# vpc-ccg/freddie

Hardware: AMD Instinct MI355X
Metric: reads segmented/sec (whole node) (higher is better)
Workload: dtype u32

## Files before the change

freddie_amd/_lib.py:

```python
import ctypes
import os

import numpy as np

from . import build as _build

_lib = None


class SegError(RuntimeError):

    def __init__(self, msg, code=None):
        super().__init__(msg)
        self.code = code


ERR_ARG, ERR_HIP, ERR_INPUT, ERR_UNSUPPORTED = 1, 2, 3, 4


class _Params(ctypes.Structure):
    _fields_ = [
        ("sigma", ctypes.c_double), ("threshold_rate", ctypes.c_double), ("variance_factor", ctypes.c_double),
        ("max_problem_size", ctypes.c_int32), ("min_read_support_outside", ctypes.c_int32),
        ("ignore_ends", ctypes.c_int32),
# ... 8 lines not shown
        ("n_part", ctypes.c_int32),
        ("part_iv_off", ctypes.c_void_p), ("iv_start", ctypes.c_void_p), ("iv_end", ctypes.c_void_p),
        ("part_rep_off", ctypes.c_void_p), ("rep_weight", ctypes.c_void_p), ("rep_exon_off", ctypes.c_void_p),
        ("ex_ts", ctypes.c_void_p), ("ex_te", ctypes.c_void_p),
    ]


class _Sizes(ctypes.Structure):
    _fields_ = [("n_final", ctypes.c_int64), ("label_bytes", ctypes.c_int64), ("n_cand", ctypes.c_int64),
                ("n_problems", ctypes.c_int64), ("n_positions", ctypes.c_int64), ("max_problem_size", ctypes.c_int64),
                ("max_problem_reads", ctypes.c_int64)]


class _Reads(ctypes.Structure):
    _fields_ = [("n_read", ctypes.c_int64)] + [(k, ctypes.c_void_p) for k in (
        "read_part", "read_rep", "strand", "seq_len", "seq_off", "read_q_off", "qs", "qe", "cig_off", "cig_op", "cig_len", "seq_classes")]


READS_DTYPES = dict(read_part=np.int32, read_rep=np.int32, strand=np.uint8, seq_len=np.int32, seq_off=np.int64, read_q_off=np.int64,
                    qs=np.int32, qe=np.int32, cig_off=np.int64, cig_op=np.uint8, cig_len=np.int32, seq_classes=np.uint32)


class _Annot(ctypes.Structure):
    _fields_ = [("n_read", ctypes.c_int64)] + [(k, ctypes.c_void_p) for k in (
        "gap_off", "gaps", "clip_off", "clips", "poly_off", "polys", "tail", "tok_off", "tok")]


EXPORTS = ["fseg_annotate", "fseg_annotation", "fseg_abi_version", "fseg_source_hash", "fseg_results", "fseg_results_packed", "fseg_create", "fseg_destroy", "fseg_last_error", "fseg_set_params", "fseg_upload",
           "fseg_run", "fseg_sync", "fseg_get_sizes", "fseg_download", "fseg_tap", "fseg_set_profiling",
           "fseg_n_stages", "fseg_stage_name", "fseg_stage_ms", "fseg_scoring_algorithmic_bytes"]

PATHS = ("small_batch", "tiny_on", "wave_on", "fuse_on", "key32", "thr_part", "label_packed", "n_solve0", "n_solve1", "n_solve2",
         "n_wide0", "n_wide1", "n_wide2", "n_tiny", "n_work", "dpw", "wide16", "known", "solve8", "tiny_kernel", "score", "arena_dp",
         "plan", "n_arena_prob", "n_score0", "n_score1", "n_score2")

TAPS = dict(pos_off=(1, np.int64), y_raw=(2, np.int32), y=(3, np.float64), threshold=(4, np.float64),
            cand_off=(5, np.int64), cand_y=(6, np.int32), fixed=(7, np.uint8), chosen=(8, np.uint8),
            final_off=(9, np.int64), final_y=(10, np.int32), problems=(11, np.int32),
            lane_start=(12, np.int32), lane_pmax=(13, np.int32), lane_exons=(14, np.int64),
            lane_stream=(15, np.int32), exon_stream=(16, np.int32), sync=(17, np.int32), paths=(18, np.int32))


def lib_path():
    return os.environ.get("FSEG_LIB") or _build.SEG_SO


def load():
    global _lib
    if _lib is not None:
        return _lib
    path = lib_path()
    if not os.path.exists(path):
        raise SegError("%s not found: build it first (freddie_amd.build.build_seg()); there is no CPU fallback" % path)
    L = ctypes.CDLL(path)
    vp = ctypes.c_void_p
    L.fseg_abi_version.restype = ctypes.c_int
    L.fseg_create.restype = ctypes.c_int
    L.fseg_create.argtypes = [ctypes.c_int, ctypes.POINTER(vp)]
    L.fseg_destroy.restype = None
    L.fseg_destroy.argtypes = [vp]
    L.fseg_last_error.restype = ctypes.c_char_p
    L.fseg_last_error.argtypes = [vp]
    L.fseg_set_params.restype = ctypes.c_int
    L.fseg_set_params.argtypes = [vp, ctypes.POINTER(_Params)]
    L.fseg_upload.restype = ctypes.c_int
    L.fseg_upload.argtypes = [vp, ctypes.POINTER(_Batch)]
    for n in ("fseg_run", "fseg_sync"):
# ... 183 lines not shown
```

freddie_amd/csrc/freddie_seg.hip:

```cpp
#include "seg_kernels.h"

using namespace fseg;

namespace {

struct DevBuf {
    void *p = nullptr;
    size_t cap = 0;
    template <typename T> T *as() const { return reinterpret_cast<T *>(p); }
};
struct Slab {
    void *p = nullptr;
    size_t cap = 0;
};
struct HostBuf {
    void *p = nullptr;
    size_t cap = 0;
    template <typename T> T *as() const { return reinterpret_cast<T *>(p); }
};
struct Carve {
    struct Item { DevBuf *b; size_t off, bytes; };
    std::vector<Item> items;
    size_t total = 0;
    size_t add(DevBuf &b, size_t bytes) {
// ... 10 lines not shown
enum Stage { ST_HIST, ST_SMOOTH, ST_THRESHOLD, ST_CANDIDATES, ST_FIX, ST_SCORE_PREP, ST_SCORE, ST_DP, ST_REFINE, ST_FINAL, ST_LABEL, ST_COUNT,
             ST_GRAPH_PRE = ST_COUNT, ST_GRAPH_POST, ST_REPORTED };
const char *kStageNames[ST_REPORTED] = {"histogram", "smooth", "threshold", "candidates", "fix_split", "scoring_prep",
                                        "interval_scoring", "dp", "refine", "final_positions", "labels", "graph_pre",
                                        "graph_post"};

enum : unsigned {
    SEG_PRE1 = 1u,
    SEG_PRE2 = 2u,
    SEG_SCORE = 4u,
    SEG_POST1 = 8u,
    SEG_POST2 = 16u,
    SEG_STATUS = 32u,
    SEG_ALL = 63u,
};

}

hipError_t fseg_sort_pairs(void *tmp, size_t *tmp_bytes, const unsigned long long *keys_in, unsigned long long *keys_out,
                           const int *vals_in, int *vals_out, size_t n, unsigned end_bit, hipStream_t stream);

struct fseg_ctx {
    int device = 0;
    hipStream_t stream = nullptr;
    std::string err;
    bool have_params = false, have_batch = false, ran = false, pending = false;
    bool fetched = false;
    fseg_params P{};
    std::vector<double> w_main, w_refine, h_table;
    int n_part = 0;
    i64 K = 0, R = 0, I = 0, NPOS = 0, LANES = 0;
    i64 max_part_pos = 0;
    int thr_part = -1;
    i64 max_part_lanes = 0;
    int n_tiles = 0;
    bool expanded = false;
    std::vector<i64> part_iv_off, part_rep_off;
    Slab slab_in, slab_pos, slab_arena;
    HostBuf h_stage;
    HostBuf h_res;
    size_t res_off[4] = {0, 0, 0, 0};
    std::vector<i64> res_pfo;
    DevBuf d_labels;
    DevBuf d_packed;
    int fetched_packed = -1;
    bool label_packed_ok = true;
    bool label_has2 = false;
    bool run_label_packed = false;
    bool labels_unpacked = false;
    DevBuf d_sort_tmp;
    DevBuf d_part_iv_off, d_part_rep_off, d_part_lane_off, d_iv_start, d_iv_end, d_pos_off, d_iv_part,
        d_rep_exon_off, d_rep_weight, d_ex_ts, d_ex_te, d_tile_desc, d_iv_tile0, d_blk_iv0, d_rb_part, d_rb_r0, d_rb_sum, d_rb_base, d_rb_max, d_rb_cmax,
        d_hc_part, d_hc_p0, d_hc_n, d_hc_glo, d_hc_ghi;
    DevBuf d_lane_ex, d_lane_start, d_lane_pmax, d_hc_llo, d_hc_lhi, d_key_a, d_key_b, d_val_a, d_val_b, d_rep_last;
    DevBuf d_lane_lx, d_lex, d_rb_esum, d_rb_ebase;
    i64 max_rep_exons = 0;
    DevBuf d_w_main, d_w_refine, d_h_table, d_thr_tab;
    DevBuf d_bits;
    DevBuf d_y_raw, d_y, d_v, d_scan_state, d_bsum, d_bsum_side, d_g, d_pk, d_pf, d_kp;
    int n_hist_chunks = 0;
    DevBuf d_voff, d_chunk_off, d_csum, d_mean, d_thr, d_label_off, d_part_has2;
    int n_rep_blocks = 0;
    DevBuf d_cand_off, d_cand_y, d_fixed0, d_added, d_fixed, d_chosen, d_final_off, d_final_y, d_final_pos, d_final_iv, d_col_thr,
        d_col_zero;
    DevBuf d_tile_defer;
    DevBuf d_blk_pre, d_tile_tot, d_seg_iv, d_seg_prev, d_rseg_c, d_cand_pn, d_cand_ll, d_cand_ln, d_cand_wide, d_prob_bs;
// ... 44 lines not shown
    static constexpr i64 kProbSelfMax = 4 * kProbBlock;
    bool prob_self_scan = false;
    i64 scan_single_max = 512;
    bool force_scan_stall = false;
    hipGraph_t graph[2] = {nullptr, nullptr};
    hipGraphExec_t graph_exec[2] = {nullptr, nullptr};
    bool profile_plain = false;
    int n_graphs = 0;
    bool last_sized = false;
    hipEvent_t ev_b[ST_COUNT] = {}, ev_e[ST_COUNT] = {};
    hipEvent_t ev_g[4] = {};
    float stage_ms[ST_REPORTED] = {};
    static constexpr int kSide = 3, kForkEvents = 32;
    hipStream_t side[kSide] = {};
    hipEvent_t fj[kForkEvents] = {};
    bool use_fork = true;
    bool force_key64 = false;
    bool wide_by_seen = false;
    char score_plan[32] = "gM|W|hB|gST";
    bool use_wave = true;
    bool use_fuse = true;
    int fuse_lanes = kFuseLanesDefault;
    bool wide_solve = true;
    bool fuse_on = true;
    bool counts_known = false;
    i64 n_solve[3] = {0, 0, 0}, n_cls_work[4] = {0, 0, 0, 0}, n_dp_cls[3] = {0, 0, 0}, n_arena_prob = 0, n_tiny = 0;
    i64 n_wide[3] = {0, 0, 0};
    i64 max_ln = 0;
    i64 tiny_from = 256;
    bool trace = false;
    bool force_global_sort = false;
    enum { PATH_SMALL_BATCH, PATH_TINY_ON, PATH_WAVE_ON, PATH_FUSE_ON, PATH_KEY32, PATH_THR_PART, PATH_LABEL_PACKED, PATH_N_SOLVE,
           PATH_N_WIDE = PATH_N_SOLVE + 3, PATH_N_TINY = PATH_N_WIDE + 3, PATH_N_WORK, PATH_DPW, PATH_WIDE16, PATH_KNOWN, PATH_SOLVE8,
           PATH_TINY_KERNEL, PATH_SCORE, PATH_ARENA_DP, PATH_PLAN, PATH_N_ARENA_PROB, PATH_N_SCORE, PATH_WORDS = PATH_N_SCORE + 3 };
    int paths[PATH_WORDS] = {};
    DevBuf d_an_in, d_an_work, d_an_out;
    HostBuf h_an_in, h_an;
    bool have_annot = false;
    fseg_annot annot{};
};

namespace {

int fail(fseg_ctx *c, int code, const char *fmt, ...) {
    char buf[512];
    va_list ap;
    va_start(ap, fmt);
    vsnprintf(buf, sizeof buf, fmt, ap);
    va_end(ap);
    if (c) c->err = buf;
    if (code == FSEG_ERR_HIP) (void)hipGetLastError();
    return code;
}
thread_local std::string g_create_error;

#define HIP_TRY(c, expr)                                                                         \
    do {                                                                                         \
        hipError_t e__ = (expr);                                                                 \
        if (e__ != hipSuccess) return fail((c), FSEG_ERR_HIP, "%s: %s", #expr, hipGetErrorString(e__)); \
    } while (0)
#define TRY(expr) do { int rc__ = (expr); if (rc__) return rc__; } while (0)

static bool g_ablate_dp = false;
static std::atomic<int> g_in_flight[64];
static std::atomic<int> g_live[64];
static std::atomic<const fseg_ctx *> g_owner[64];
static void set_in_flight(fseg_ctx *c, bool on);
// ... 196 lines not shown
    };
    auto launch_fork_waiters = [&]() {
        if (!dev_sync) return;
        for (int k = 1; k < ps.n_seg; ++k) if (dev_side(k))
            hipLaunchKernelGGL(k_wait_word, dim3(1), dim3(64), 0, c->side[ps.side_of[k]], st, &sw->emit_gen, 1u, sync_gen, kSyncTicks);
    };
    const i64 avg_len = NPOS / (K > 0 ? K : 1);
    const int iv_threads = avg_len > 65536 ? 1024 : (avg_len > 16384 ? 256 : 64);
    int tile_grid = grid_for(c->n_tiles, 1, 16384);
    const i64 scan_nb = scan_blocks(NPOS);
    const int scan_grid = scan_nb > 0 ? (int)scan_nb : 1;
    u64 *scan_state = c->d_scan_state.as<u64>();
    const bool scan_single = scan_nb <= c->scan_single_max;
    int *bsum = scan_single ? nullptr : c->d_bsum.as<int>();
    int *bsum_side = scan_single ? nullptr : c->d_bsum_side.as<int>();
    auto scan_counts = [&](hipStream_t q, int *bs, const unsigned *flags, u64 *total_dev, i64 *off_last) {
        if (scan_single) return;
        hipLaunchKernelGGL(k_scan1, dim3(grid_for(scan_nb, 1, 4096)), dim3(256), 0, q, flags, NPOS, bs);
        hipLaunchKernelGGL(k_scan2, dim3(1), dim3(kScan2Threads), 0, q, bs, scan_nb, total_dev, off_last);
    };
    int work_grid = grid_for(c->work_cap, 1, 4096);
    ProblemArrays pr{c->d_prob_iv.as<int>(), c->d_prob_start.as<int>(), c->d_prob_n.as<int>(),
                     c->d_prob_pair_off.as<i64>(), c->d_prob_tri_off.as<i64>(), c->d_prob_flags.as<int>(),
                     c->d_prob_chain.as<int>(), c->d_prob_cov_off.as<i64>(), c->d_prob_lane_lo.as<int>(),
                     c->d_prob_lane_n.as<int>()};
    const int pg = grid_for(NPOS / 8 / kProbBlock + 1, 1, 1024);
    i64 *prob_bs = (c->prob_self_scan && !sized) ? nullptr : c->d_prob_bs.as<i64>();
    if (do_pre1) {
    {
        const i64 nw = 3 * (i64)flag_words(NPOS);
        hipLaunchKernelGGL(k_clear, dim3(grid_for(nw / 4 + 1, 256, 2048)), dim3(256), 0, s, st, c->d_bits.as<unsigned>(), nw);
    }
    begin(ST_HIST);
    hipLaunchKernelGGL(k_hist, dim3(grid_for(c->n_hist_chunks, 1, 16384)), dim3(512), 0, s, c->n_hist_chunks,
                       c->d_hc_part.as<int>(), c->d_hc_p0.as<i64>(), c->d_hc_n.as<int>(), c->d_hc_glo.as<int>(),
                       c->d_hc_ghi.as<int>(), c->d_hc_llo.as<i64>(), c->d_hc_lhi.as<i64>(), c->d_part_iv_off.as<i64>(), c->d_iv_start.as<int>(), c->d_iv_end.as<int>(),
                       c->d_pos_off.as<i64>(), c->d_part_lane_off.as<i64>(), c->d_lane_lx.as<int2>(),
                       c->d_lane_start.as<int>(), c->d_lane_pmax.as<int>(),
                       c->d_lex.as<int2>(), c->P.ignore_ends, c->d_y_raw.as<int>(), st,
                       scan_state, scan_single ? scan_nb * 3 : 0);
    end(ST_HIST); begin(ST_SMOOTH);
#define FSEG_LAUNCH_SMOOTH(RV)                                                                                         \
    hipLaunchKernelGGL(k_smooth<RV>, dim3(tile_grid), dim3(kSmoothThreads), 0, s, c->n_tiles, c->d_tile_desc.as<TileDesc>(),      \
                       c->d_y_raw.as<int>(), c->d_w_main.as<double>(),                                                 \
                       c->P.radius_main, c->d_y.as<double>(), flag_pos_bits,                           \
                       flag_cand_bits, c->d_blk_pre.as<int>(), c->d_tile_tot.as<int>(), c->d_tile_defer.as<int>())
    if (c->P.radius_main == 20) { FSEG_LAUNCH_SMOOTH(20); }
    else if (c->P.radius_main == 12) { FSEG_LAUNCH_SMOOTH(12); }
    else { FSEG_LAUNCH_SMOOTH(0); }
#undef FSEG_LAUNCH_SMOOTH
    end(ST_SMOOTH);
    {
    hipStream_t q = fork(0);
    if (stage_events && c->profile_all) (void)hipEventRecord(c->ev_b[ST_THRESHOLD], q);
    const bool thr_part_fits = c->max_part_pos <= (i64)kThrPartMaxChunks * 8192;
    const bool thr_part = thr_part_fits && (c->thr_part == 1 || (c->thr_part < 0 && n_part >= 64));
    if (thr_part) {
        c->paths[fseg_ctx::PATH_THR_PART] = 1;
        hipLaunchKernelGGL(k_thr_part, dim3(grid_for(n_part, 1, 4096)), dim3(512), 0, q, n_part, c->d_part_iv_off.as<i64>(), c->d_pos_off.as<i64>(), NPOS,
                           flag_pos_bits, c->d_y.as<double>(), c->d_v.as<double>(), c->P.variance_factor, c->d_mean.as<double>(), c->d_thr.as<double>());
    } else {
    c->paths[fseg_ctx::PATH_THR_PART] = 0;
    scan_counts(q, bsum_side, flag_pos_bits, &st->n_vals, nullptr);
    hipLaunchKernelGGL(k_scan_emit<kEmitValues>, dim3(scan_grid), dim3(256), 0, q, flag_pos_bits, NPOS,
                       bsum_side, scan_state, &st->n_vals, (i64 *)nullptr, &st->err, c->d_y.as<double>(), c->d_v.as<double>(), K, c->d_pos_off.as<i64>(),
                       c->d_iv_start.as<int>(), c->d_blk_iv0.as<int>(), (int *)nullptr, (int *)nullptr, (i64 *)nullptr,
                       c->force_scan_stall ? 1 : 0, (int *)nullptr);
    hipLaunchKernelGGL(k_voff, dim3(grid_for(n_part + 1, 1, 2048)), dim3(64), 0, q, n_part, c->d_part_iv_off.as<i64>(),
                       c->d_pos_off.as<i64>(), NPOS, flag_pos_bits, bsum_side, scan_state, &st->n_vals,
                       c->d_voff.as<i64>());
    hipLaunchKernelGGL(k_vplan, dim3(1), dim3(256), 0, q, n_part, c->d_part_iv_off.as<i64>(), c->d_pos_off.as<i64>(), NPOS,
                       c->d_voff.as<i64>(), c->d_chunk_off.as<i64>(), st, c->chunk_cap);
    int chunk_grid = grid_for(c->chunk_cap, 1, 4096);
// ... 43 lines not shown
    begin(ST_SCORE_PREP);
    hipLaunchKernelGGL(k_prob_emit, dim3(pg), dim3(256), 0, s, st, c->d_cand_pn.as<int>(), c->d_cand_ll.as<int>(),
                       c->d_cand_ln.as<int>(), c->d_seg_iv.as<int>(), c->d_cand_off.as<i64>(), prob_bs,
                       pr, c->prob_cap, c->d_work_pc.as<int2>(), c->d_cls_items.as<int4>(),
                       c->work_cap, c->d_dp_items.as<int>(), c->d_prob_desc.as<ProbDesc>(), c->d_iv_start.as<int>(),
                       c->d_iv_part.as<int>(), c->d_part_lane_off.as<i64>(), split, c->d_solve_items.as<int>(), c->d_solve_desc.as<ProbDesc>(),
                       c->d_wide_items.as<int>(), c->d_wide_all.as<int>(), c->d_cand_wide.as<unsigned char>(),
                       dev_sync ? sw : (SyncWords *)nullptr, sync_gen);
    launch_fork_waiters();
    if (c->prob_cap > 0 && any_arena) {
        if (stage_events && do_score) { end(ST_SCORE_PREP); begin(ST_SCORE); score_begun = true; }
        const int cov_blocks = work_grid < 2048 ? work_grid : 2048;
        const int pt_blocks = c->small_batch ? grid_for(c->prob_cap, 1, 512) : 0;
        if (!pt_blocks)
            hipLaunchKernelGGL(k_pair_thresholds, dim3(grid_for(c->prob_cap, 1, 2048)), dim3(256), 0, s, st, pr,
                               c->d_prob_desc.as<ProbDesc>(), c->prob_cap, c->d_cand_off.as<i64>(), c->d_cand_y.as<int>(),
                               c->d_h_table.as<double>(), c->P.h_len,
                               c->P.threshold_rate, c->d_pair_thr.as<int2>(), c->pair_cap, c->d_amb.as<unsigned>(),
                               c->d_out.as<unsigned>(), c->tri_cap);
        hipLaunchKernelGGL(k_cov, dim3(cov_blocks + pt_blocks), dim3(kLaneChunk), 0, s, st,
                           c->d_prob_desc.as<ProbDesc>(), c->prob_cap, c->d_work_pc.as<int2>(), c->work_cap, c->d_cand_off.as<i64>(),
                           c->d_cand_y.as<int>(), c->d_iv_start.as<int>(), c->d_lane_lx.as<int2>(),
                           c->d_lex.as<int2>(),
                           c->d_cov.as<unsigned>(), c->cov_cap, c->d_work_active.as<unsigned char>(),
                           cov_blocks, pr, c->d_h_table.as<double>(), c->P.h_len, c->P.threshold_rate, c->d_pair_thr.as<int2>(),
                           c->pair_cap, c->d_amb.as<unsigned>(), c->d_out.as<unsigned>(), c->tri_cap);
    }
    if (!score_begun) end(ST_SCORE_PREP);
    }
    if (do_score && !score_begun) begin(ST_SCORE);
    int *const census = c->paths;
    if (do_score) {
        for (int w = 0; w < fseg_ctx::PATH_WORDS; ++w)
            if (w != fseg_ctx::PATH_THR_PART && w != fseg_ctx::PATH_LABEL_PACKED && w != fseg_ctx::PATH_ARENA_DP) census[w] = 0;
        census[fseg_ctx::PATH_SMALL_BATCH] = c->small_batch; census[fseg_ctx::PATH_TINY_ON] = c->tiny_on; census[fseg_ctx::PATH_WAVE_ON] = wave;
        census[fseg_ctx::PATH_FUSE_ON] = c->use_fuse && c->fuse_on; census[fseg_ctx::PATH_KNOWN] = known; census[fseg_ctx::PATH_PLAN] = plan != nullptr;
    }
    if (do_score && c->prob_cap > 0) {
        const bool sfork = any_arena;
        hipStream_t qt = (tiny_max > 0 && sfork) ? fork(2) : s;
#ifdef FSEG_SCORE_TIMING
#define FSEG_TARG , c->d_tacc.as<unsigned long long>()
#else
#define FSEG_TARG
#endif
#ifndef FSEG_WG_SMALL
#define FSEG_WG_SMALL 4096
#endif
#ifndef FSEG_WG_MID
#define FSEG_WG_MID 2048
#endif
#ifndef FSEG_WG_TINY
#define FSEG_WG_TINY 4096
#endif
#define FSEG_LAUNCH_SCORE(Q, NMV, CLS, MAXWG)                                                                           \
        do { note_score(CLS);                                                                                                  \
        hipLaunchKernelGGL(k_score<NMV>, dim3(work_grid < (MAXWG) ? work_grid : (MAXWG)), dim3(ScoreCfg<NMV>::kThreads),  \
                           score_lds_for((NMV) == kNMax ? c->nm_big : (NMV), (NMV) + 1), Q, st, CLS,                                 \
                           ((NMV) == kNMax ? c->nm_big : (NMV)), pr, c->prob_cap, c->d_cls_items.as<int4>(),              \
                           c->d_prob_desc.as<ProbDesc>(), c->work_cap, c->d_cand_off.as<i64>(),                         \
                           c->d_cand_y.as<int>(), c->d_work_active.as<unsigned char>(), c->d_cov.as<unsigned>(),        \
                           c->cov_cap, c->d_pair_thr.as<int2>(), c->pair_cap, c->d_out.as<unsigned>(), c->tri_cap,      \
                           c->d_amb.as<unsigned>() FSEG_TARG); } while (0)
        auto wide_n = [&](int cls, size_t cnt_bytes) -> i64 { return (known && cls >= 0 && cls < 3 && cnt_bytes == 2) ? c->n_wide[cls] : -1; };
#define FSEG_SOLVE_N(CNT, CLS, N_ITEMS) (wide_n(CLS, sizeof(CNT)) >= 0 ? wide_n(CLS, sizeof(CNT)) : (i64)(N_ITEMS))
#define FSEG_SOLVE_WIDE(CNT, CLS) (wide_n(CLS, sizeof(CNT)) >= 0 ? c->d_wide_items.as<int>() : (const int *)nullptr)
#define FSEG_SOLVE_ARGS(NMV, CNT, CLS)                                                                                      \
// ... 645 lines not shown
        e = hipFuncSetAttribute(reinterpret_cast<const void *>(k_score_huge), hipFuncAttributeMaxDynamicSharedMemorySize,
                                (int)kHugeScoreLds);
    {
        auto lds_attr = [&](const void *f, size_t bytes) { if (e == hipSuccess) e = hipFuncSetAttribute(f, hipFuncAttributeMaxDynamicSharedMemorySize, (int)bytes); };
        lds_attr(reinterpret_cast<const void *>(k_solve<kNMax, unsigned char, int, false>), solve_lds_for(kNMax, kNMax + 1, 1));
        lds_attr(reinterpret_cast<const void *>(k_solve<kNMax, unsigned char, i64, false>), solve_lds_for(kNMax, kNMax + 1, 1));
        lds_attr(reinterpret_cast<const void *>(k_solve<kNMax, unsigned short, int, false>), solve_lds_for(kNMax, kNMax + 1, 2));
        lds_attr(reinterpret_cast<const void *>(k_solve<kNMax, unsigned short, i64, false>), solve_lds_for(kNMax, kNMax + 1, 2));
        lds_attr(reinterpret_cast<const void *>(k_solve<kNMax, unsigned char, int, true>), solve_lds_for(kNMax, kNMax + 1, 1));
        lds_attr(reinterpret_cast<const void *>(k_solve<kNMax, unsigned short, int, true>), solve_lds_for(kNMax, kNMax + 1, 2));
        lds_attr(reinterpret_cast<const void *>(k_dpw<kNMax, unsigned char, int, 64>), dpw_lds_for(kNMax, 4, 1));
        lds_attr(reinterpret_cast<const void *>(k_dpw<kNMax, unsigned short, int, 64>), dpw_lds_for(kNMax, 4, 2));
        lds_attr(reinterpret_cast<const void *>(k_dpw<kNMax, unsigned char, i64, 64>), dpw_lds_for(kNMax, 8, 1));
        lds_attr(reinterpret_cast<const void *>(k_dpw<kNMax, unsigned short, i64, 64>), dpw_lds_for(kNMax, 8, 2));
        lds_attr(reinterpret_cast<const void *>(k_dpw<kNMax, unsigned char, int, 512>), dpw_lds_for(kNMax, 4, 1));
        lds_attr(reinterpret_cast<const void *>(k_dpw<kNMax, unsigned short, int, 512>), dpw_lds_for(kNMax, 4, 2));
        lds_attr(reinterpret_cast<const void *>(k_dpw<kNMax, unsigned char, i64, 512>), dpw_lds_for(kNMax, 8, 1));
        lds_attr(reinterpret_cast<const void *>(k_dpw<kNMax, unsigned short, i64, 512>), dpw_lds_for(kNMax, 8, 2));
    }
    if (e == hipSuccess)
        e = hipFuncSetAttribute(reinterpret_cast<const void *>(k_dp_huge), hipFuncAttributeMaxDynamicSharedMemorySize,
                                (int)kHugeDpLds);
    if (e != hipSuccess) {
        g_create_error = std::string("context creation failed: ") + hipGetErrorString(e);
        if (c->counted_live) g_live[device].fetch_sub(1);
        delete c;
        return FSEG_ERR_HIP;
    }
    c->d_status.cap = sizeof(Status); c->d_prep.cap = sizeof(PrepStatus); c->d_tacc.cap = kTaccBytes; c->d_sync.cap = sizeof(SyncWords);
    auto flag = [](const char *name) { const char *v = getenv(name); return v && v[0] == '1'; };
    { const char *v = getenv("FSEG_DEV_SYNC"); if (v && v[0] == '0') c->dev_sync = false; }
    if (flag("FSEG_LABEL_BYTES")) c->label_packed_ok = false;
    { const char *v = getenv("FSEG_THR_PART"); if (v && (v[0] == '0' || v[0] == '1')) c->thr_part = v[0] - '0'; }
    { const char *v = getenv("FSEG_SYNC_TICKS"); if (v && v[0] && atoll(v) > 0) c->sync_ticks = (unsigned)atoll(v); }
    if (flag("FSEG_NO_GRAPH")) c->use_graph = false;
    if (flag("FSEG_NO_FORK")) c->use_fork = false;
    if (flag("FSEG_NO_FUSE")) c->use_fuse = false;
    if (flag("FSEG_NO_WAVE")) c->use_wave = false;
    if (flag("FSEG_FORCE_KEY64")) c->force_key64 = true;
    if (flag("FSEG_WIDE_BY_SEEN")) c->wide_by_seen = true;
    if (const char *e = getenv("FSEG_SPLIT_DP")) c->split_dp = atoi(e) & 15;
    if (const char *e = getenv("FSEG_SCORE_PLAN")) snprintf(c->score_plan, sizeof c->score_plan, "%s", e);
    {
        int seen[4] = {0, 0, 0, 0};
        static const char kinds[] = "BMST";
        for (const char *q = c->score_plan; *q; ++q) { const char *at = strchr(kinds, *q); if (at) ++seen[at - kinds]; }
        int bars = 0;
        for (const char *q = c->score_plan; *q; ++q) bars += *q == '|';
        if (seen[0] != 1 || seen[1] != 1 || seen[2] != 1 || seen[3] != 1 || bars > fseg_ctx::kSide) c->score_plan[0] = 0;
    }
    { const char *v = getenv("FSEG_FUSE_LANES"); if (v && v[0] && atoi(v) > 0 && atoi(v) <= kFuseLanesWide) c->fuse_lanes = atoi(v); }
    if (flag("FSEG_NO_SIZED")) c->use_sized = false;
    if (flag("FSEG_TRACE")) c->trace = true;
    if (flag("FSEG_GLOBAL_SORT")) c->force_global_sort = true;
    if (flag("FSEG_FORCE_SCAN_STALL")) c->force_scan_stall = true;
    { const char *tf = getenv("FSEG_TINY_FROM"); if (tf && tf[0]) c->tiny_from = atoll(tf); }
    { const char *sm = getenv("FSEG_SCAN_SINGLE_MAX"); if (sm && sm[0]) c->scan_single_max = atoll(sm); }
    *out = c;
    return FSEG_OK;
}

void fseg_destroy(fseg_ctx *c) {
    if (!c) return;
    set_in_flight(c, false);
    release_device(c);
    if (c->counted_live) { g_live[c->device].fetch_sub(1); c->counted_live = false; }
// ... 72 lines not shown
    const i64 K = b->part_iv_off[np], R = b->part_rep_off[np];
    if (b->part_iv_off[0] != 0 || b->part_rep_off[0] != 0 || b->rep_exon_off[0] != 0)
        return fail(c, FSEG_ERR_ARG, "fseg_upload: offsets must start at 0");
    if (K <= 0 || R < 0) return fail(c, FSEG_ERR_ARG, "fseg_upload: bad offsets");
    const i64 I = b->rep_exon_off[R];
    if (I < 0) return fail(c, FSEG_ERR_ARG, "rep_exon_off not monotone");
    if (I >= 0x7fffffffLL) return fail(c, FSEG_ERR_UNSUPPORTED, "batch has %lld exons; split it (limit 2^31-1 per upload)", (long long)I);
    i64 NPOS = 0, n_tiles = 0, lanes = 0, n_rep_blocks = 0, max_part_reps = 0, max_rep_exons = 0;
    bool expanded = false;
    for (int p = 0; p < np; ++p) {
        const i64 k0 = b->part_iv_off[p], k1 = b->part_iv_off[p + 1];
        if (k1 <= k0) return fail(c, FSEG_ERR_INPUT, "partition %d has no intervals", p);
        if (b->part_rep_off[p + 1] < b->part_rep_off[p]) return fail(c, FSEG_ERR_ARG, "part_rep_off not monotone");
        for (i64 k = k0; k < k1; ++k) {
            if (!(b->iv_start[k] < b->iv_end[k])) return fail(c, FSEG_ERR_INPUT, "partition %d: interval with start >= end (py/freddie_segment.py:140)", p);
            if (k > k0 && !(b->iv_end[k - 1] < b->iv_start[k])) return fail(c, FSEG_ERR_INPUT, "partition %d: intervals overlap or are unordered (py/freddie_segment.py:138)", p);
            const i64 len = (i64)b->iv_end[k] - b->iv_start[k] + 1;
            NPOS += len;
            n_tiles += (len + kSmoothTile - 1) / kSmoothTile;
        }
        n_rep_blocks += (b->part_rep_off[p + 1] - b->part_rep_off[p] + 255) / 256;
        if (b->part_rep_off[p + 1] - b->part_rep_off[p] > max_part_reps) max_part_reps = b->part_rep_off[p + 1] - b->part_rep_off[p];
    }
    if (NPOS >= 0x7fffffffLL) return fail(c, FSEG_ERR_UNSUPPORTED, "batch has %lld positions; split it (limit 2^31-1 per upload)", (long long)NPOS);
    for (i64 r = 0; r < R; ++r) {
        const int w = b->rep_weight[r];
        if (w < 1) return fail(c, FSEG_ERR_INPUT, "rep %lld has weight %d (< 1)", (long long)r, w);
        if (w != 1) expanded = true;
        lanes += w;
        if (b->rep_exon_off[r + 1] < b->rep_exon_off[r]) return fail(c, FSEG_ERR_ARG, "rep_exon_off not monotone");
        if (b->rep_exon_off[r + 1] - b->rep_exon_off[r] > max_rep_exons) max_rep_exons = b->rep_exon_off[r + 1] - b->rep_exon_off[r];
    }
    if (lanes >= 0x7fffffffLL) return fail(c, FSEG_ERR_UNSUPPORTED, "batch has %lld reads; split it (limit 2^31-1 per upload)", (long long)lanes);
    int hist_chunk = kHistChunk;
    while (hist_chunk > 1024 && NPOS / hist_chunk < 512) hist_chunk >>= 1;
    i64 n_chunks = 0;
    {
        i64 k = 0, pos = 0;
        for (int p = 0; p < np; ++p) {
            i64 Pp = 0;
            for (k = b->part_iv_off[p]; k < b->part_iv_off[p + 1]; ++k) Pp += (i64)b->iv_end[k] - b->iv_start[k] + 1;
            n_chunks += (Pp + hist_chunk - 1) / hist_chunk;
            pos += Pp;
        }
        (void)pos;
    }
    const i64 nb = scan_blocks(NPOS);
    if (n_tiles >= 0x7fffffffLL || n_chunks >= 0x7fffffffLL) return fail(c, FSEG_ERR_UNSUPPORTED, "batch too large");
    Carve in;
    in.add(c->d_part_iv_off, ((size_t)np + 1) * 8);
    in.add(c->d_part_rep_off, ((size_t)np + 1) * 8);
    in.add(c->d_part_lane_off, ((size_t)np + 1) * 8);
    in.add(c->d_iv_start, (size_t)K * 4);
    in.add(c->d_iv_end, (size_t)K * 4);
    in.add(c->d_pos_off, ((size_t)K + 1) * 8);
    in.add(c->d_iv_part, (size_t)K * 4);
    in.add(c->d_iv_tile0, (size_t)K * 4);
    in.add(c->d_tile_desc, (size_t)n_tiles * sizeof(TileDesc));
    in.add(c->d_blk_iv0, ((size_t)nb + 1) * 4);
    in.add(c->d_rb_part, (size_t)n_rep_blocks * 4);
    in.add(c->d_rb_r0, (size_t)n_rep_blocks * 4);
    in.add(c->d_hc_part, (size_t)n_chunks * 4);
    in.add(c->d_hc_p0, (size_t)n_chunks * 8);
    in.add(c->d_hc_n, (size_t)n_chunks * 4);
    in.add(c->d_hc_glo, (size_t)n_chunks * 4);
    in.add(c->d_hc_ghi, (size_t)n_chunks * 4);
    in.add(c->d_rep_exon_off, ((size_t)R + 1) * 8);
// ... 48 lines not shown
            }
            for (i64 r = b->part_rep_off[p]; r < b->part_rep_off[p + 1]; r += 256) { h_rb_part[rb] = p; h_rb_r0[rb] = (int)r; ++rb; }
            for (i64 r = b->part_rep_off[p]; r < b->part_rep_off[p + 1]; ++r) l += b->rep_weight[r];
            h_lane_off[p + 1] = l;
            if (l - h_lane_off[p] > c->max_part_lanes) c->max_part_lanes = l - h_lane_off[p];
            const i64 P0 = h_pos_off[k0], P1 = h_pos_off[k1];
            if (P1 - P0 > c->max_part_pos) c->max_part_pos = P1 - P0;
            i64 k = k0;
            for (i64 q0 = P0; q0 < P1; q0 += hist_chunk) {
                const i64 q1 = std::min<i64>(q0 + hist_chunk, P1) - 1;
                while (h_pos_off[k + 1] <= q0) ++k;
                i64 kk = k;
                while (h_pos_off[kk + 1] <= q1) ++kk;
                h_hc_part[ch] = p; h_hc_p0[ch] = q0; h_hc_n[ch] = (int)(q1 - q0 + 1);
                h_hc_glo[ch] = b->iv_start[k] + (int)(q0 - h_pos_off[k]);
                h_hc_ghi[ch] = b->iv_start[kk] + (int)(q1 - h_pos_off[kk]);
                ++ch;
            }
        }
        h_blk[nb] = (int)(K - 1);
    }
    const double t_tables = tk.ms();
    memcpy(host_of(c->d_part_iv_off), b->part_iv_off, ((size_t)np + 1) * 8);
    memcpy(host_of(c->d_part_rep_off), b->part_rep_off, ((size_t)np + 1) * 8);
    memcpy(host_of(c->d_iv_start), b->iv_start, (size_t)K * 4);
    memcpy(host_of(c->d_iv_end), b->iv_end, (size_t)K * 4);
    memcpy(host_of(c->d_rep_exon_off), b->rep_exon_off, ((size_t)R + 1) * 8);
    memcpy(host_of(c->d_rep_weight), b->rep_weight, (size_t)R * 4);
    memcpy(host_of(c->d_ex_ts), b->ex_ts, (size_t)I * 4);
    memcpy(host_of(c->d_ex_te), b->ex_te, (size_t)I * 4);
    const double t_copy = tk.ms();
    c->n_part = np; c->K = K; c->R = R; c->I = I; c->NPOS = NPOS; c->LANES = lanes; c->expanded = expanded;
    if (c->max_part_lanes > lanes) c->max_part_lanes = lanes;
    c->n_tiles = (int)n_tiles; c->n_hist_chunks = (int)n_chunks; c->n_rep_blocks = (int)n_rep_blocks; c->max_rep_exons = max_rep_exons;
    c->part_iv_off.assign(b->part_iv_off, b->part_iv_off + np + 1);
    c->part_rep_off.assign(b->part_rep_off, b->part_rep_off + np + 1);
    hipStream_t s = c->stream;
    HIP_TRY(c, hipMemcpyAsync(c->slab_in.p, stage, up_bytes, hipMemcpyHostToDevice, s));
    {
        PrepStatus init;
        init.err = 0; init.pad = 0;
        for (int q = 0; q < 4; ++q) init.bad_rep[q] = 0x7fffffffffffffffLL;
        *c->h_prep = init;
        HIP_TRY(c, hipMemcpyAsync(c->d_prep.p, c->h_prep, sizeof(PrepStatus), hipMemcpyHostToDevice, s));
        c->prep_checked = false;
    }
    if (R > 0) {
        hipLaunchKernelGGL(k_prep_reps, dim3(grid_for(n_rep_blocks, 1, 65536)), dim3(256), 0, s, (int)n_rep_blocks, c->d_rb_part.as<int>(),
                           c->d_rb_r0.as<int>(), c->d_part_rep_off.as<i64>(), c->d_part_iv_off.as<i64>(), c->d_iv_start.as<int>(),
                           c->d_iv_end.as<int>(), c->d_rep_exon_off.as<i64>(), c->d_ex_ts.as<int>(), c->d_ex_te.as<int>(),
                           c->d_key_a.as<u64>(), c->d_val_a.as<int>(), c->d_rep_last.as<int>(), c->d_prep.as<PrepStatus>());
        const bool sort_here = max_part_reps <= kLaneSortMax && !c->force_global_sort;
        if (!sort_here) {
            unsigned end_bit = 33;
            while (end_bit < 64 && ((u64)np >> (end_bit - 32)) != 0) ++end_bit;
            size_t tmp_bytes = 0;
            HIP_TRY(c, fseg_sort_pairs(nullptr, &tmp_bytes, c->d_key_a.as<u64>(), c->d_key_b.as<u64>(), c->d_val_a.as<int>(), c->d_val_b.as<int>(),
                                       (size_t)R, end_bit, s));
            TRY(ensure(c, c->d_sort_tmp, tmp_bytes));
            HIP_TRY(c, fseg_sort_pairs(c->d_sort_tmp.p, &tmp_bytes, c->d_key_a.as<u64>(), c->d_key_b.as<u64>(), c->d_val_a.as<int>(),
                                       c->d_val_b.as<int>(), (size_t)R, end_bit, s));
        }
        if (sort_here) {
            hipLaunchKernelGGL(k_lanes, dim3(grid_for(np, 1, 65536)), dim3(256), 0, s, np, c->d_part_rep_off.as<i64>(), c->d_part_lane_off.as<i64>(),
                               c->d_key_b.as<u64>(), c->d_val_b.as<int>(), c->d_rep_weight.as<int>(), c->d_rep_last.as<int>(),
                               c->d_rep_exon_off.as<i64>(), c->d_lane_ex.as<longlong2>(), c->d_lane_start.as<int>(), c->d_lane_pmax.as<int>(),
                               1, c->d_key_a.as<u64>(), c->d_ex_ts.as<int>(), c->d_ex_te.as<int>(), c->d_lane_lx.as<int2>(), c->d_lex.as<int2>());
// ... 624 lines not shown
```

freddie_amd/csrc/seg_common.h:

```cpp
#pragma once
#include <hip/hip_runtime.h>
#include <type_traits>
#include <hsa/hsa.h>
#include <hsa/hsa_ext_amd.h>
#include <chrono>
#include <algorithm>
#include <atomic>
#include <mutex>
#include <cmath>
#include <cstdarg>
#include <cstdio>
#include <cstdlib>
#include <cstring>
#include <string>
#include <vector>

#include "freddie_seg.h"

namespace fseg {


typedef long long i64;

typedef unsigned long long u64;
// ... 141 lines not shown
    if (i < 0) i += p;
    return i < n ? i : p - 1 - i;
}


__device__ __forceinline__ void label_thresholds(i64 L, const double *h_table, int h_len, double tau, int *hi_out,
                                                 int *lo_out) {
    double h = L < (i64)h_len ? h_table[L] : tau;
    double l = 1.0 - h;
    double dL = (double)L;
    i64 v = (i64)floor(h * dL);
    if (v < 0) v = 0;
    while (v > 0 && (double)(v - 1) / dL > h) --v;
    while (!((double)v / dL > h) && v <= L + 1) ++v;
    *hi_out = (int)v;
    i64 u = (i64)ceil(l * dL);
    if (u > L) u = L;
    while (u >= 0 && !((double)u / dL < l)) --u;
    while ((double)(u + 1) / dL < l && u < L) ++u;
    *lo_out = (int)u;
}


constexpr int kThrTab = 8192;

__device__ __forceinline__ void label_thresholds_tab(i64 L, const int2 *tab, const double *h_table, int h_len, double tau,
                                                     int *hi_out, int *lo_out) {
    if (L < (i64)kThrTab) { const int2 t = tab[L]; *hi_out = t.x; *lo_out = t.y; }
    else label_thresholds(L, h_table, h_len, tau, hi_out, lo_out);
}


constexpr int kHistChunk = 8192;

constexpr int kHistIv = 1024;


template <int NW = 0> __device__ __forceinline__ int wg_exclusive_scan(int v, int *lds, int *total);


__device__ __forceinline__ void lds_barrier() {
    __builtin_amdgcn_fence(__ATOMIC_RELEASE, "workgroup", "local");
    __builtin_amdgcn_s_barrier();
    __builtin_amdgcn_fence(__ATOMIC_ACQUIRE, "workgroup", "local");
}

template <int NW = 0>
__device__ __forceinline__ int wg_exclusive_scan_lds(int v, int *lds , int *total) {
    int lane = threadIdx.x & 63, wave = threadIdx.x >> 6;
    const int nw = NW > 0 ? NW : (int)((blockDim.x + 63) >> 6);
    int x = v;
    for (int d = 1; d < 64; d <<= 1) {
        int y = __shfl_up(x, d);
        if (lane >= d) x += y;
    }
    lds_barrier();
    if (lane == 63) lds[wave] = x;
    lds_barrier();
    int off = 0, tot = 0;
    for (int w = 0; w < nw; ++w) {
        int sv = lds[w];
        if (w < wave) off += sv;
        tot += sv;
    }
    *total = tot;
    return off + x - v;
// ... 1031 lines not shown
```

freddie_amd/csrc/seg_front.hip:

```cpp
#include "seg_kernels.h"

#include <type_traits>

namespace fseg {

__global__ void __launch_bounds__(256) k_thr_table(const double *h_table, int h_len, double tau, int2 *tab) {
    for (int L = blockIdx.x * blockDim.x + threadIdx.x; L < kThrTab; L += gridDim.x * blockDim.x) {
        int hi = 0x7fffffff, lo = -1;
        if (L >= 1) label_thresholds((i64)L, h_table, h_len, tau, &hi, &lo);
        tab[L] = make_int2(hi, lo);
    }
}

__global__ void __launch_bounds__(512) k_hist(int n_chunks, const int *chunk_part, const i64 *chunk_p0, const int *chunk_n,
                                              const int *chunk_glo, const int *chunk_ghi, const i64 *chunk_lane_lo,
                                              const i64 *chunk_lane_hi, const i64 *part_iv_off,
                                              const int *iv_start, const int *iv_end, const i64 *pos_off,
                                              const i64 *part_lane_off, const int2 *__restrict__ lane_lx, const int *lane_start,
                                              const int *lane_pmax, const int2 *__restrict__ lex,
                                              int ignore_ends, int *y_raw, Status *st, u64 *zero_ptr, i64 zero_n) {
    __shared__ int hist[kHistChunk];
    __shared__ int ivs_s[kHistIv], ive_s[kHistIv], base_s[kHistIv];
    for (i64 i = (i64)blockIdx.x * blockDim.x + threadIdx.x; i < zero_n; i += (i64)gridDim.x * blockDim.x) zero_ptr[i] = 0;
    for (int ch = blockIdx.x; ch < n_chunks; ch += gridDim.x) {
        const int part = chunk_part[ch];
        const i64 p0 = chunk_p0[ch];
        const int np = chunk_n[ch];
        const int g_lo = chunk_glo[ch], g_hi = chunk_ghi[ch];
        const i64 k0 = part_iv_off[part], k1 = part_iv_off[part + 1];
        __syncthreads();
        for (int i = threadIdx.x; i < np; i += blockDim.x) hist[i] = 0;
        const i64 lo = chunk_lane_lo[ch], hi = chunk_lane_hi[ch];
        const int nk = (int)(k1 - k0);
        const bool cached = nk <= kHistIv;
        if (cached)
            for (int i = threadIdx.x; i < nk; i += blockDim.x) {
                ivs_s[i] = iv_start[k0 + i]; ive_s[i] = iv_end[k0 + i];
                base_s[i] = (int)(pos_off[k0 + i] - p0) - iv_start[k0 + i];
            }
        __syncthreads();
        const int sub = threadIdx.x & 7;
        const int G8 = blockDim.x >> 3;
        auto count_exon = [&](i64 e, i64 e0, i64 e1, int ts, int te) {
            if (te < g_lo || ts > g_hi) return;
            int kl = 0;
            bool ok;
            int base;
            if (cached) {
                int a2 = 0, b2 = nk;
                while (b2 - a2 > 1) { int m = (a2 + b2) >> 1; if (ivs_s[m] <= ts) a2 = m; else b2 = m; }
                kl = a2;
                ok = ts >= ivs_s[kl] && ts <= ive_s[kl] && te <= ive_s[kl];
                base = base_s[kl];
            } else {
                ok = ts >= iv_start[k0];
                i64 k = k0;
                if (ok) { k = k0 + last_le(iv_start + k0, k1 - k0, ts); ok = ts <= iv_end[k] && te <= iv_end[k]; }
                base = (int)(pos_off[k] - p0) - iv_start[k];
            }
            if (!ok) { atomicOr(&st->err, kErrExonInterval); return; }
            if (!(ignore_ends && e == e0) && ts >= g_lo && ts <= g_hi) atomicAdd(&hist[base + ts], 1);
            if (!(ignore_ends && e == e1 - 1) && te >= g_lo && te <= g_hi) atomicAdd(&hist[base + te], 1);
        };
        for (i64 l0 = lo + (threadIdx.x >> 3); l0 < hi; l0 += 4 * (i64)G8) {
            int2 ex[4], x0[4];
#pragma unroll
            for (int u = 0; u < 4; ++u) { const i64 l = l0 + (i64)u * G8; ex[u] = lane_lx[l < hi ? l : l0]; }
#pragma unroll
            for (int u = 0; u < 4; ++u) {
                const int e = ex[u].x + sub < ex[u].y ? ex[u].x + sub : ex[u].x;
                x0[u] = lex[e];
            }
#pragma unroll
            for (int u = 0; u < 4; ++u) {
                if (l0 + (i64)u * G8 >= hi) break;
                const i64 e0 = ex[u].x, e1 = ex[u].y;
                if (e0 + sub < e1) count_exon(e0 + sub, e0, e1, x0[u].x, x0[u].y);
                for (i64 e = e0 + sub + 8; e < e1; e += 8) { const int2 x = lex[e]; count_exon(e, e0, e1, x.x, x.y); }
            }
        }
        __syncthreads();
        for (int i = threadIdx.x; i < np; i += blockDim.x) y_raw[p0 + i] = hist[i];
    }
}

template <int R>
#ifndef FSEG_SMOOTH_OCC
#define FSEG_SMOOTH_OCC 6
#endif
__global__ void __launch_bounds__(kSmoothThreads, FSEG_SMOOTH_OCC) k_smooth(int n_tiles, const TileDesc *__restrict__ tiles,
                                                const int *__restrict__ y_raw, const double *__restrict__ w_g, int radius_rt,
                                                double *y_out, unsigned *flag_pos, unsigned *flag_cand, int *blk_pre, int *tile_tot,
                                                int *tile_defer) {
    __shared__ int xs[kSmoothTile + 2 * kMaxRadius];
    __shared__ unsigned tw_c[kSmoothTile / 32 + 1], tw_p[kSmoothTile / 32 + 1];
    __shared__ int defer_s;
    __shared__ int blk_s[kSmoothTile / kSumBlock];
    __shared__ double ws[kMaxRadius + 1];
    __shared__ double ys[kSmoothTile];
    const int radius = R > 0 ? R : radius_rt;
    const int span = kSmoothTile + 2 * radius;
    constexpr int kStage = R > 0 ? (kSmoothTile + 2 * R + kSmoothThreads - 1) / kSmoothThreads : kSmoothStage;
    for (int j = threadIdx.x; j <= radius; j += blockDim.x) ws[j] = w_g[j];
    const int G = gridDim.x;
    auto load_counts = [&](const TileDesc &d, int *v) {
        const int len_d = __builtin_amdgcn_readfirstlane(d.len), y0_d = __builtin_amdgcn_readfirstlane(d.y0);
        const int yb = y0_d - radius + (int)threadIdx.x;
        const int *src = y_raw + (((i64)__builtin_amdgcn_readfirstlane((int)(d.base >> 32)) << 32) | (unsigned)__builtin_amdgcn_readfirstlane((int)d.base));
        if (R > 0 && y0_d + kSmoothTile + radius <= len_d) {
            static_assert(R <= kSmoothThreads, "a tile's left halo lies in the first staged element of each thread");
#pragma unroll
            for (int e = 0; e < kStage; ++e) {
                const int idx = e * kSmoothThreads + threadIdx.x;
                const int y = yb + e * kSmoothThreads;
                const int r = e == 0 && y < 0 ? -1 - y : y;
// ... 488 lines not shown
__global__ void k_vsum_part(int n_part, const i64 *voff, const i64 *chunk_off, const double *csum0, const double *csum1,
                            double vf, double *mean, double *thr, i64 chunk_cap) {
    for (int p = blockIdx.x * blockDim.x + threadIdx.x; p < n_part; p += gridDim.x * blockDim.x) {
        i64 c0 = chunk_off[p], c1 = chunk_off[p + 1];
        if (c1 > chunk_cap) c1 = chunk_cap;
        double n = (double)(voff[p + 1] - voff[p]);
        double s0 = 0.0, s1 = 0.0;
        for (i64 c = c0; c < c1; ++c) {
            s0 = (c == c0) ? csum0[c] : __dadd_rn(s0, csum0[c]);
            s1 = (c == c0) ? csum1[c] : __dadd_rn(s1, csum1[c]);
        }
        const double mu = s0 / n;
        mean[p] = mu;
        thr[p] = __dadd_rn(mu, __dmul_rn(vf, __dsqrt_rn(s1 / n)));
    }
}

__global__ void __launch_bounds__(256) k_peaks_edges(int n_tiles, const TileDesc *tiles, const int *tile_defer, const double *x,
                                                     unsigned *flag, int *part_has2, int n_part) {
    if (blockIdx.x == 0) for (int p = threadIdx.x; p < n_part; p += blockDim.x) part_has2[p] = 0;
    for (int t = blockIdx.x * blockDim.x + threadIdx.x; t < n_tiles; t += gridDim.x * blockDim.x) {
        const TileDesc d = tiles[t];
        const i64 first = d.base + d.y0, last = d.base + d.len - 1;
        const i64 tile_last = first + kSmoothTile - 1;
        if (d.y0 > 0 && first < last) peak_from(first, last, x, flag);
        if (tile_last < last && kSmoothTile > 1) peak_from(tile_last, last, x, flag);
        const int df = tile_defer[t];
        if (df >= 0) peak_from(first + df, last, x, flag);
    }
}


__attribute__((used)) static const void *const kInstances[] = {
    reinterpret_cast<const void *>(&k_smooth<20>),
    reinterpret_cast<const void *>(&k_smooth<12>),
    reinterpret_cast<const void *>(&k_smooth<0>),
    reinterpret_cast<const void *>(&k_scan_emit<kEmitValues>),
    reinterpret_cast<const void *>(&k_scan_emit<kEmitPositions>),
};

}
```

freddie_amd/csrc/seg_kernels.h:

```cpp
#pragma once
#include "seg_common.h"

namespace fseg {

__global__ void __launch_bounds__(256) k_thr_table(const double *h_table, int h_len, double tau, int2 *tab);

__global__ void __launch_bounds__(512) k_hist(int n_chunks, const int *chunk_part, const i64 *chunk_p0, const int *chunk_n,
                                              const int *chunk_glo, const int *chunk_ghi, const i64 *chunk_lane_lo,
                                              const i64 *chunk_lane_hi, const i64 *part_iv_off,
                                              const int *iv_start, const int *iv_end, const i64 *pos_off,
                                              const i64 *part_lane_off, const int2 *__restrict__ lane_lx, const int *lane_start,
                                              const int *lane_pmax, const int2 *__restrict__ lex,
                                              int ignore_ends, int *y_raw, Status *st, u64 *zero_ptr, i64 zero_n);

template <int R>
#ifndef FSEG_SMOOTH_OCC
#define FSEG_SMOOTH_OCC 6
#endif
__global__ void __launch_bounds__(kSmoothThreads, FSEG_SMOOTH_OCC) k_smooth(int n_tiles, const TileDesc *__restrict__ tiles,
                                                const int *__restrict__ y_raw, const double *__restrict__ w_g, int radius_rt,
                                                double *y_out, unsigned *flag_pos, unsigned *flag_cand, int *blk_pre, int *tile_tot,
                                                int *tile_defer);

__global__ void __launch_bounds__(256) k_clear(Status *st, unsigned *bits, i64 n_words);

__global__ void __launch_bounds__(256) k_scan1(const unsigned *flags, i64 n, int *bsum);

__global__ void __launch_bounds__(kScan2Threads) k_scan2(int *bsum, i64 nb, u64 *total_out, i64 *off_last );

template <int MODE>
__global__ void __launch_bounds__(256) k_scan_emit(const unsigned *flags, i64 n, const int *bsum ,
                                                   u64 *state, u64 *total_out, i64 *off_last ,
                                                   unsigned *err, const double *y,
                                                   double *v, i64 K, const i64 *pos_off, const int *iv_start,
                                                   const int *blk_iv0, int *out_y, int *out_pos, i64 *out_off,
                                                   int force_stall , int *out_iv );

__global__ void __launch_bounds__(64) k_voff(int n_part, const i64 *part_iv_off, const i64 *pos_off, i64 n_pos,
                                             const unsigned *flags, const int *bsum , const u64 *state, const u64 *total, i64 *voff);
// ... 229 lines not shown
```

Baseline: 577.6 million.

## Pack histogram counters into 16-bit halves to double shared-memory chunk size

Adds a templated k_hist variant that stores two 16-bit position counters per shared-memory word, which allows a 16384-position chunk in the same LDS footprint. The host checks at upload whether any partition could exceed 65535 overlapping exon ends (via a sort of weighted endpoints) and falls back to 32-bit counters if so. Larger chunks mean fewer chunks and less per-chunk overhead (interval caching, zeroing), and zeroing uses 16-byte stores. The cost is a host-side sort per large partition during upload, plus extra unpacking on write-out.

```diff
diff --git a/freddie_amd/_lib.py b/freddie_amd/_lib.py
--- a/freddie_amd/_lib.py
+++ b/freddie_amd/_lib.py
@@ -64,7 +64,7 @@
 
 PATHS = ("small_batch", "tiny_on", "wave_on", "fuse_on", "key32", "thr_part", "label_packed", "n_solve0", "n_solve1", "n_solve2",
          "n_wide0", "n_wide1", "n_wide2", "n_tiny", "n_work", "dpw", "wide16", "known", "solve8", "tiny_kernel", "score", "arena_dp",
-         "plan", "n_arena_prob", "n_score0", "n_score1", "n_score2")
+         "plan", "n_arena_prob", "n_score0", "n_score1", "n_score2", "hist16")
 
 TAPS = dict(pos_off=(1, np.int64), y_raw=(2, np.int32), y=(3, np.float64), threshold=(4, np.float64),
             cand_off=(5, np.int64), cand_y=(6, np.int32), fixed=(7, np.uint8), chosen=(8, np.uint8),
diff --git a/freddie_amd/csrc/freddie_seg.hip b/freddie_amd/csrc/freddie_seg.hip
--- a/freddie_amd/csrc/freddie_seg.hip
+++ b/freddie_amd/csrc/freddie_seg.hip
@@ -66,6 +66,8 @@
     i64 K = 0, R = 0, I = 0, NPOS = 0, LANES = 0;
     i64 max_part_pos = 0;
     int thr_part = -1;
+    int hist16 = -1;
+    bool hist_packed = false;
     i64 max_part_lanes = 0;
     int n_tiles = 0;
     bool expanded = false;
@@ -176,7 +178,7 @@
     bool force_global_sort = false;
     enum { PATH_SMALL_BATCH, PATH_TINY_ON, PATH_WAVE_ON, PATH_FUSE_ON, PATH_KEY32, PATH_THR_PART, PATH_LABEL_PACKED, PATH_N_SOLVE,
            PATH_N_WIDE = PATH_N_SOLVE + 3, PATH_N_TINY = PATH_N_WIDE + 3, PATH_N_WORK, PATH_DPW, PATH_WIDE16, PATH_KNOWN, PATH_SOLVE8,
-           PATH_TINY_KERNEL, PATH_SCORE, PATH_ARENA_DP, PATH_PLAN, PATH_N_ARENA_PROB, PATH_N_SCORE, PATH_WORDS = PATH_N_SCORE + 3 };
+           PATH_TINY_KERNEL, PATH_SCORE, PATH_ARENA_DP, PATH_PLAN, PATH_N_ARENA_PROB, PATH_N_SCORE, PATH_HIST16 = PATH_N_SCORE + 3, PATH_WORDS };
     int paths[PATH_WORDS] = {};
     DevBuf d_an_in, d_an_work, d_an_out;
     HostBuf h_an_in, h_an;
@@ -439,13 +441,18 @@
         hipLaunchKernelGGL(k_clear, dim3(grid_for(nw / 4 + 1, 256, 2048)), dim3(256), 0, s, st, c->d_bits.as<unsigned>(), nw);
     }
     begin(ST_HIST);
-    hipLaunchKernelGGL(k_hist, dim3(grid_for(c->n_hist_chunks, 1, 16384)), dim3(512), 0, s, c->n_hist_chunks,
-                       c->d_hc_part.as<int>(), c->d_hc_p0.as<i64>(), c->d_hc_n.as<int>(), c->d_hc_glo.as<int>(),
-                       c->d_hc_ghi.as<int>(), c->d_hc_llo.as<i64>(), c->d_hc_lhi.as<i64>(), c->d_part_iv_off.as<i64>(), c->d_iv_start.as<int>(), c->d_iv_end.as<int>(),
-                       c->d_pos_off.as<i64>(), c->d_part_lane_off.as<i64>(), c->d_lane_lx.as<int2>(),
-                       c->d_lane_start.as<int>(), c->d_lane_pmax.as<int>(),
-                       c->d_lex.as<int2>(), c->P.ignore_ends, c->d_y_raw.as<int>(), st,
-                       scan_state, scan_single ? scan_nb * 3 : 0);
+#define FSEG_LAUNCH_HIST(BITS)                                                                                         \
+    hipLaunchKernelGGL(k_hist<BITS>, dim3(grid_for(c->n_hist_chunks, 1, 16384)), dim3(512), 0, s, c->n_hist_chunks,   \
+                       c->d_hc_part.as<int>(), c->d_hc_p0.as<i64>(), c->d_hc_n.as<int>(), c->d_hc_glo.as<int>(),       \
+                       c->d_hc_ghi.as<int>(), c->d_hc_llo.as<i64>(), c->d_hc_lhi.as<i64>(), c->d_part_iv_off.as<i64>(), c->d_iv_start.as<int>(), c->d_iv_end.as<int>(), \
+                       c->d_pos_off.as<i64>(), c->d_part_lane_off.as<i64>(), c->d_lane_lx.as<int2>(),                  \
+                       c->d_lane_start.as<int>(), c->d_lane_pmax.as<int>(),                                            \
+                       c->d_lex.as<int2>(), c->P.ignore_ends, c->d_y_raw.as<int>(), st,                                \
+                       scan_state, scan_single ? scan_nb * 3 : 0)
+    c->paths[fseg_ctx::PATH_HIST16] = c->hist_packed;
+    if (c->hist_packed) { FSEG_LAUNCH_HIST(16); }
+    else { FSEG_LAUNCH_HIST(32); }
+#undef FSEG_LAUNCH_HIST
     end(ST_HIST); begin(ST_SMOOTH);
 #define FSEG_LAUNCH_SMOOTH(RV)                                                                                         \
     hipLaunchKernelGGL(k_smooth<RV>, dim3(tile_grid), dim3(kSmoothThreads), 0, s, c->n_tiles, c->d_tile_desc.as<TileDesc>(),      \
@@ -555,7 +562,7 @@
     int *const census = c->paths;
     if (do_score) {
         for (int w = 0; w < fseg_ctx::PATH_WORDS; ++w)
-            if (w != fseg_ctx::PATH_THR_PART && w != fseg_ctx::PATH_LABEL_PACKED && w != fseg_ctx::PATH_ARENA_DP) census[w] = 0;
+            if (w != fseg_ctx::PATH_THR_PART && w != fseg_ctx::PATH_LABEL_PACKED && w != fseg_ctx::PATH_ARENA_DP && w != fseg_ctx::PATH_HIST16) census[w] = 0;
         census[fseg_ctx::PATH_SMALL_BATCH] = c->small_batch; census[fseg_ctx::PATH_TINY_ON] = c->tiny_on; census[fseg_ctx::PATH_WAVE_ON] = wave;
         census[fseg_ctx::PATH_FUSE_ON] = c->use_fuse && c->fuse_on; census[fseg_ctx::PATH_KNOWN] = known; census[fseg_ctx::PATH_PLAN] = plan != nullptr;
     }
@@ -1267,6 +1274,7 @@
     { const char *v = getenv("FSEG_DEV_SYNC"); if (v && v[0] == '0') c->dev_sync = false; }
     if (flag("FSEG_LABEL_BYTES")) c->label_packed_ok = false;
     { const char *v = getenv("FSEG_THR_PART"); if (v && (v[0] == '0' || v[0] == '1')) c->thr_part = v[0] - '0'; }
+    { const char *v = getenv("FSEG_HIST16"); if (v && (v[0] == '0' || v[0] == '1')) c->hist16 = v[0] - '0'; }
     { const char *v = getenv("FSEG_SYNC_TICKS"); if (v && v[0] && atoll(v) > 0) c->sync_ticks = (unsigned)atoll(v); }
     if (flag("FSEG_NO_GRAPH")) c->use_graph = false;
     if (flag("FSEG_NO_FORK")) c->use_fork = false;
@@ -1405,7 +1413,27 @@
         if (b->rep_exon_off[r + 1] - b->rep_exon_off[r] > max_rep_exons) max_rep_exons = b->rep_exon_off[r + 1] - b->rep_exon_off[r];
     }
     if (lanes >= 0x7fffffffLL) return fail(c, FSEG_ERR_UNSUPPORTED, "batch has %lld reads; split it (limit 2^31-1 per upload)", (long long)lanes);
-    int hist_chunk = kHistChunk;
+    bool hist_packed = c->hist16 != 0;
+    for (int p = 0; p < np && hist_packed; ++p) {
+        const i64 r0 = b->part_rep_off[p], r1 = b->part_rep_off[p + 1];
+        i64 part_lanes = 0;
+        for (i64 r = r0; r < r1; ++r) part_lanes += b->rep_weight[r];
+        if (2 * part_lanes <= kHistCountMax16) continue;
+        std::vector<std::pair<int, int>> ends;
+        ends.reserve((size_t)(2 * (b->rep_exon_off[r1] - b->rep_exon_off[r0])));
+        for (i64 r = r0; r < r1; ++r)
+            for (i64 e = b->rep_exon_off[r]; e < b->rep_exon_off[r + 1]; ++e) {
+                ends.emplace_back(b->ex_ts[e], b->rep_weight[r]);
+                ends.emplace_back(b->ex_te[e], b->rep_weight[r]);
+            }
+        std::sort(ends.begin(), ends.end());
+        i64 count = 0;
+        for (size_t i = 0; i < ends.size() && hist_packed; ++i) {
+            count = (i > 0 && ends[i].first == ends[i - 1].first ? count : 0) + ends[i].second;
+            if (count > kHistCountMax16) hist_packed = false;
+        }
+    }
+    int hist_chunk = hist_packed ? kHistChunk16 : kHistChunk;
     while (hist_chunk > 1024 && NPOS / hist_chunk < 512) hist_chunk >>= 1;
     i64 n_chunks = 0;
     {
@@ -1520,7 +1548,7 @@
     const double t_copy = tk.ms();
     c->n_part = np; c->K = K; c->R = R; c->I = I; c->NPOS = NPOS; c->LANES = lanes; c->expanded = expanded;
     if (c->max_part_lanes > lanes) c->max_part_lanes = lanes;
-    c->n_tiles = (int)n_tiles; c->n_hist_chunks = (int)n_chunks; c->n_rep_blocks = (int)n_rep_blocks; c->max_rep_exons = max_rep_exons;
+    c->n_tiles = (int)n_tiles; c->n_hist_chunks = (int)n_chunks; c->hist_packed = hist_packed; c->n_rep_blocks = (int)n_rep_blocks; c->max_rep_exons = max_rep_exons;
     c->part_iv_off.assign(b->part_iv_off, b->part_iv_off + np + 1);
     c->part_rep_off.assign(b->part_rep_off, b->part_rep_off + np + 1);
     hipStream_t s = c->stream;
diff --git a/freddie_amd/csrc/seg_common.h b/freddie_amd/csrc/seg_common.h
--- a/freddie_amd/csrc/seg_common.h
+++ b/freddie_amd/csrc/seg_common.h
@@ -197,6 +197,12 @@
 
 
 constexpr int kHistChunk = 8192;
+#ifndef FSEG_HIST_CHUNK16
+#define FSEG_HIST_CHUNK16 16384
+#endif
+constexpr int kHistChunk16 = FSEG_HIST_CHUNK16;
+static_assert(kHistChunk16 % 8 == 0, "the packed counters are zeroed sixteen bytes at a time");
+constexpr int kHistCountMax16 = 65535;
 
 constexpr int kHistIv = 1024;
 
diff --git a/freddie_amd/csrc/seg_front.hip b/freddie_amd/csrc/seg_front.hip
--- a/freddie_amd/csrc/seg_front.hip
+++ b/freddie_amd/csrc/seg_front.hip
@@ -12,6 +12,7 @@
     }
 }
 
+template <int BITS>
 __global__ void __launch_bounds__(512) k_hist(int n_chunks, const int *chunk_part, const i64 *chunk_p0, const int *chunk_n,
                                               const int *chunk_glo, const int *chunk_ghi, const i64 *chunk_lane_lo,
                                               const i64 *chunk_lane_hi, const i64 *part_iv_off,
@@ -19,7 +20,10 @@
                                               const i64 *part_lane_off, const int2 *__restrict__ lane_lx, const int *lane_start,
                                               const int *lane_pmax, const int2 *__restrict__ lex,
                                               int ignore_ends, int *y_raw, Status *st, u64 *zero_ptr, i64 zero_n) {
-    __shared__ int hist[kHistChunk];
+    static_assert(BITS == 32 || BITS == 16, "a counter is a word or half a word");
+    using Word = std::conditional_t<BITS == 16, unsigned, int>;
+    constexpr int kWords = BITS == 16 ? kHistChunk16 / 2 : kHistChunk;
+    __shared__ __attribute__((aligned(16))) Word hist[kWords];
     __shared__ int ivs_s[kHistIv], ive_s[kHistIv], base_s[kHistIv];
     for (i64 i = (i64)blockIdx.x * blockDim.x + threadIdx.x; i < zero_n; i += (i64)gridDim.x * blockDim.x) zero_ptr[i] = 0;
     for (int ch = blockIdx.x; ch < n_chunks; ch += gridDim.x) {
@@ -29,7 +33,11 @@
         const int g_lo = chunk_glo[ch], g_hi = chunk_ghi[ch];
         const i64 k0 = part_iv_off[part], k1 = part_iv_off[part + 1];
         __syncthreads();
-        for (int i = threadIdx.x; i < np; i += blockDim.x) hist[i] = 0;
+        if constexpr (BITS == 16) {
+            for (int i = threadIdx.x; i < (np + 7) >> 3; i += blockDim.x) reinterpret_cast<uint4 *>(hist)[i] = make_uint4(0u, 0u, 0u, 0u);
+        } else {
+            for (int i = threadIdx.x; i < np; i += blockDim.x) hist[i] = 0;
+        }
         const i64 lo = chunk_lane_lo[ch], hi = chunk_lane_hi[ch];
         const int nk = (int)(k1 - k0);
         const bool cached = nk <= kHistIv;
@@ -41,6 +49,10 @@
         __syncthreads();
         const int sub = threadIdx.x & 7;
         const int G8 = blockDim.x >> 3;
+        auto hit = [&](int i) {
+            if constexpr (BITS == 16) atomicAdd(&hist[i >> 1], 1u << (16 * (i & 1)));
+            else atomicAdd(&hist[i], 1);
+        };
         auto count_exon = [&](i64 e, i64 e0, i64 e1, int ts, int te) {
             if (te < g_lo || ts > g_hi) return;
             int kl = 0;
@@ -59,8 +71,8 @@
                 base = (int)(pos_off[k] - p0) - iv_start[k];
             }
             if (!ok) { atomicOr(&st->err, kErrExonInterval); return; }
-            if (!(ignore_ends && e == e0) && ts >= g_lo && ts <= g_hi) atomicAdd(&hist[base + ts], 1);
-            if (!(ignore_ends && e == e1 - 1) && te >= g_lo && te <= g_hi) atomicAdd(&hist[base + te], 1);
+            if (!(ignore_ends && e == e0) && ts >= g_lo && ts <= g_hi) hit(base + ts);
+            if (!(ignore_ends && e == e1 - 1) && te >= g_lo && te <= g_hi) hit(base + te);
         };
         for (i64 l0 = lo + (threadIdx.x >> 3); l0 < hi; l0 += 4 * (i64)G8) {
             int2 ex[4], x0[4];
@@ -80,7 +92,18 @@
             }
         }
         __syncthreads();
-        for (int i = threadIdx.x; i < np; i += blockDim.x) y_raw[p0 + i] = hist[i];
+        if constexpr (BITS == 16) {
+            const int odd = (int)(p0 & 1);
+            auto count_at = [&](int i) { return (int)((hist[i >> 1] >> (16 * (i & 1))) & 0xffffu); };
+            for (int i0 = 2 * (int)threadIdx.x - odd; i0 < np; i0 += 2 * (int)blockDim.x) {
+                const int i1 = i0 + 1;
+                if (i0 >= 0 && i1 < np) *reinterpret_cast<int2 *>(y_raw + p0 + i0) = make_int2(count_at(i0), count_at(i1));
+                else if (i0 >= 0) y_raw[p0 + i0] = count_at(i0);
+                else y_raw[p0 + i1] = count_at(i1);
+            }
+        } else {
+            for (int i = threadIdx.x; i < np; i += blockDim.x) y_raw[p0 + i] = hist[i];
+        }
     }
 }
 
@@ -635,6 +658,8 @@
 
 
 __attribute__((used)) static const void *const kInstances[] = {
+    reinterpret_cast<const void *>(&k_hist<32>),
+    reinterpret_cast<const void *>(&k_hist<16>),
     reinterpret_cast<const void *>(&k_smooth<20>),
     reinterpret_cast<const void *>(&k_smooth<12>),
     reinterpret_cast<const void *>(&k_smooth<0>),
diff --git a/freddie_amd/csrc/seg_kernels.h b/freddie_amd/csrc/seg_kernels.h
--- a/freddie_amd/csrc/seg_kernels.h
+++ b/freddie_amd/csrc/seg_kernels.h
@@ -5,6 +5,7 @@
 
 __global__ void __launch_bounds__(256) k_thr_table(const double *h_table, int h_len, double tau, int2 *tab);
 
+template <int BITS>
 __global__ void __launch_bounds__(512) k_hist(int n_chunks, const int *chunk_part, const i64 *chunk_p0, const int *chunk_n,
                                               const int *chunk_glo, const int *chunk_ghi, const i64 *chunk_lane_lo,
                                               const i64 *chunk_lane_hi, const i64 *part_iv_off,
```

After: 589.4 million, median of 6. +2.0%, better.
